# ishine/TTS-3

Measured on AMD Instinct MI355X. Metric: audio samples/sec + RTF, HiFiGAN-v1 22.05kHz 80-mel, batch 32 @ 1/2/4/8 GPU, higher is better.
Workload: dtype fp32 (power-of-2 scaled fp16 hi/lo split on fp16 MFMA, fp32 accumulate); 1 GPU; HiFiGAN-v1 22.05kHz inference, [32,80,1024] mel per GPU (replicate pad 5), fp32; model=HiFiGAN-v1 (hifigan_config.py generator_model_params), global_batch=32, seq_len=1024, parallelism=dp1 (utterance sharding; no collectives)

## Files before the change

tts-3_amd/csrc/kernels_resblock.hip:

```cpp
#include <algorithm>
#include <cstdlib>
#include <type_traits>

#include "resblock_block.hpp"
#include "split_device.hpp"

namespace tts {




constexpr int kPostK = 7;
constexpr int kPostHalo = 3;

template <class S, int K, int C, int PD, int GEO, bool ALLX = false, bool POST = false>
struct PairCfg {
  static constexpr int RP_W = (GEO == 0 || GEO == 4 || GEO == 5 || GEO == 7) ? 256 : (GEO == 1 ? 192 : 128);
  static constexpr int LEAD = (K - 1) / 2;
  static constexpr int RP_BN = RP_W - 2 * LEAD;
  static constexpr int NW = GEO >= 5 ? 8 : 4;
  static constexpr int NT = 64 * NW;
  static constexpr int WN = (GEO == 0 || GEO == 5) ? 4 : (GEO == 8 ? 1 : 2);
  static constexpr int WM = NW / WN;
  static constexpr int TM = C / 32 / WM;
// ... 186 lines not shown

  const int xrow0 = wn * TN * 32 + l32;
  auto read_x = [&](const unsigned char* xl, int k, f32x4 (*dst)[NP]) {
#pragma unroll
    for (int n = 0; n < TN; ++n) {
      const unsigned char* p = xl + (xrow0 + n * 32 + k * d) * S::ROWB + 16 * half;
#pragma unroll
      for (int q = 0; q < NP; ++q) dst[n][q] = *reinterpret_cast<const f32x4*>(p + 32 * q);
    }
  };

  if constexpr (ALLX) {
#pragma unroll
    for (int c = 0; c < NC; ++c) load_x(c);
#pragma unroll
    for (int c = 0; c < NC; ++c) store_x(c, c);
  } else {
    load_x(0);
    store_x(0, 0);
  }
  if (tid < C) {
    bsm[tid] = bias1;
    bsm[C + tid] = bias2;
  }
  if constexpr (POST)
    for (int e = tid; e < C * kPostK; e += NT) pws[e] = pa.post_w[e];
  __syncthreads();
#pragma unroll
  for (int c = 0; c < NC; ++c) {
    const unsigned char* xl = smem + (ALLX ? c : (c & 1)) * P::XSZB;
    if (!ALLX && c + 1 < NC) load_x(c + 1);
    read_x(xl, 0, bcur);
#pragma unroll
    for (int k = 0; k < K; ++k) {
      const int s = c * K + k;
#pragma unroll
      for (int m = 0; m < TM; ++m)
#pragma unroll
        for (int q = 0; q < NP; ++q) ar[PD][m][q] = bload4(ra[m], avoff, (unsigned)((s + PD) * NP + q) * 1024u);
      if (k + 1 < K) read_x(xl, k + 1, bnext);
      __builtin_amdgcn_sched_barrier(0);
      mfma_step();
      if (k + 1 < K) {
#pragma unroll
        for (int n = 0; n < TN; ++n)
#pragma unroll
          for (int q = 0; q < NP; ++q) bcur[n][q] = bnext[n][q];
      }
    }
    if (!ALLX && c + 1 < NC) store_x((c + 1) & 1, c + 1);
    if (!ALLX || c + 1 == NC) __syncthreads();
  }

  {
    const float sc1 = H3 ? ldexpf(1.f, ex + a1.w_exp) : 1.f;
    float tmax = 0.f;
#pragma unroll
    for (int m = 0; m < TM; ++m) {
      float bv[16];
#pragma unroll
      for (int r = 0; r < 16; ++r) bv[r] = bsm[mrow0 + m * 32 + (r & 3) + 8 * (r >> 2) + 4 * half];
#pragma unroll
      for (int n = 0; n < TN; ++n) {
        const int t = tx0 + xrow0 + n * 32;
        const bool inside = t >= 0 && t < T;
#pragma unroll
        for (int r = 0; r < 16; ++r) {
          float v = lrelu2(acc[m][n][r] * sc1 + bv[r], a1.out_slope);
          v = inside ? v : 0.f;
          acc[m][n][r] = v;
          tmax = fmaxf(tmax, fabsf(v));
        }
      }
    }
    float tscale = 1.f;
    int et = 0;
    if (H3) {
      tmax = wave_max(tmax);
      if (lane == 0) red[wave] = tmax;
      __syncthreads();
      float mx = red[0];
#pragma unroll
      for (int w = 1; w < P::NW; ++w) mx = fmaxf(mx, red[w]);
      if (mx > 0.f && mx < INFINITY) {
        int E;
        (void)frexpf(mx, &E);
        et = E - 14;
      }
      tscale = ldexpf(1.f, -et);
    }
#pragma unroll
    for (int m = 0; m < TM; ++m)
#pragma unroll
      for (int n = 0; n < TN; ++n)
#pragma unroll
        for (int gl = 0; gl < 2; ++gl)
          store_xt8<S>(smem + (((mrow0 + m * 32) / 16 + gl) * P::TROWS + xrow0 + n * 32) * S::ROWB + 16 * half,
                       acc[m][n], 8 * gl, tscale);
    constexpr int ZB = (P::TROWS - RP_W) * S::ROWB;
    for (int e = tid * 16; e < NC * ZB; e += NT * 16) {
      const int g = e / ZB;
      *reinterpret_cast<f32x4*>(smem + (g * P::TROWS + RP_W) * S::ROWB + (e - g * ZB)) = f32x4{};
    }
    __syncthreads();
    const Conv1dArgs& a2 = pa.c2;
#pragma unroll
    for (int m = 0; m < TM; ++m) ra[m] = make_rsrc(a2.w + ((size_t)(wm * TM + m) * NC * K) * (NP * 256), 0xFFFFFFFFu);
#pragma unroll
    for (int m = 0; m < TM; ++m)
#pragma unroll
      for (int n = 0; n < TN; ++n) acc[m][n] = f32x16{};
#pragma unroll
    for (int p = 0; p < PD; ++p)
#pragma unroll
      for (int m = 0; m < TM; ++m)
#pragma unroll
        for (int q = 0; q < NP; ++q) ar[p][m][q] = bload4(ra[m], avoff, (unsigned)(p * NP + q) * 1024u);
    const int trow0 = xrow0;
    auto read_t = [&](int g, int k, f32x4 (*dst)[NP]) {
#pragma unroll
      for (int n = 0; n < TN; ++n) {
        const unsigned char* p = smem + (g * P::TROWS + trow0 + n * 32 + k) * S::ROWB + 16 * half;
#pragma unroll
        for (int q = 0; q < NP; ++q) dst[n][q] = *reinterpret_cast<const f32x4*>(p + 32 * q);
      }
    };
    read_t(0, 0, bcur);
#pragma unroll
    for (int g = 0; g < NC; ++g) {
#pragma unroll
      for (int k = 0; k < K; ++k) {
        const int s = g * K + k;
#pragma unroll
        for (int m = 0; m < TM; ++m)
#pragma unroll
          for (int q = 0; q < NP; ++q) ar[PD][m][q] = bload4(ra[m], avoff, (unsigned)((s + PD) * NP + q) * 1024u);
        const bool more = (k + 1 < K) || (g + 1 < NC);
        if (more) read_t((k + 1 < K) ? g : g + 1, (k + 1 < K) ? k + 1 : 0, bnext);
        __builtin_amdgcn_sched_barrier(0);
        mfma_step();
        if (more) {
#pragma unroll
          for (int n = 0; n < TN; ++n)
#pragma unroll
            for (int q = 0; q < NP; ++q) bcur[n][q] = bnext[n][q];
        }
      }
    }
    if (H3) {
      const float sc2 = ldexpf(1.f, et + a2.w_exp);
#pragma unroll
      for (int m = 0; m < TM; ++m)
#pragma unroll
        for (int n = 0; n < TN; ++n) acc[m][n] *= sc2;
    }
    if constexpr (POST) {
      post_epilogue(pa, acc, b, t0, mrow0, wn, lane);
    } else {
      conv_epilogue<TM, TN, H3, YB>(a2, acc, b, t0 + wn * TN * 32, mrow0, lane, t0 + RP_BN, bsm + C);
    }
  }
}

namespace {
template <class S, int K, int C, int GEO>
void launch_pair_t(const ResPairArgs& a, int B, hipStream_t s) {
  constexpr bool AX = C == 64 && GEO != 2;
  constexpr int PD = S::NP == 1 ? RES_PD_B1 : 2;
  auto go = [&](auto pl_tag) {
    constexpr int PL = decltype(pl_tag)::value;
    if (a.post_w) {
      using P = PairCfg<S, K, C, PD, GEO, AX, true>;
      static_assert(P::RP_BN - 2 * kPostHalo <= 256, "one conv_post column per thread");
      dim3 grid(ceil_div(a.c1.Tout, P::STRIDE), 1, B);
      hipLaunchKernelGGL((resblock_pair_kernel<S, K, C, PD, GEO, AX, true, PL>), grid, dim3(P::NT), 0, s, a);
      return;
    }
    using P = PairCfg<S, K, C, PD, GEO, AX>;
    dim3 grid(ceil_div(a.c1.Tout, P::RP_BN), 1, B);
    hipLaunchKernelGGL((resblock_pair_kernel<S, K, C, PD, GEO, AX, false, PL>), grid, dim3(P::NT), 0, s, a);
  };
  if (a.c1.planes != 0) {
    constexpr bool OK = std::is_same<S, SchemeB1>::value;
    TTS_REQUIRE(OK && a.c1.planes == (kPlaneXB16 | kPlaneYB16) && a.c2.planes == a.c1.planes, 3,
                "resblock pair: bf16 planes need the bf16 scheme");
    if constexpr (OK) go(std::integral_constant<int, kPlaneXB16 | kPlaneYB16>{});
    return;
  }
  go(std::integral_constant<int, 0>{});
}

int pair_geo64() {
  static const int g = [] {
    const char* e = std::getenv("TTS_MI355X_PAIR_GEO64");
    return e && std::atoi(e) == 2 ? 2 : (e && std::atoi(e) == 4 ? 4 : 1);
  }();
  return g;
}

template <class S, int K>
void launch_pair_k(const ResPairArgs& a, int B, int C, hipStream_t s) {
  if constexpr (S::NP == 1) {
    if (C == 128) {
      static const int geo = [] {
        const char* e = std::getenv("TTS_MI355X_PAIR128_GEO");
        return e && e[0] == '2' ? 2 : (e && e[0] == '0' ? 0 : (e && e[0] == '4' ? 4 : (e && e[0] == '5' ? 5 : 7)));
      }();
      if (geo == 2) launch_pair_t<S, K, 128, 2>(a, B, s);
      else if (geo == 7) launch_pair_t<S, K, 128, 7>(a, B, s);
      else if (geo == 5) launch_pair_t<S, K, 128, 5>(a, B, s);
      else if (geo == 4) launch_pair_t<S, K, 128, 4>(a, B, s);
      else launch_pair_t<S, K, 128, 0>(a, B, s);
      return;
    }
    if (C == 256) {
      static const int geo = [] {
        const char* e = std::getenv("TTS_MI355X_PAIR256_GEO");
        return e && e[0] == '2' ? 2 : (e && e[0] == '6' ? 6 : 8);
      }();
      if (geo == 6) launch_pair_t<S, K, 256, 6>(a, B, s);
      else if (geo == 8) launch_pair_t<S, K, 256, 8>(a, B, s);
      else launch_pair_t<S, K, 256, 2>(a, B, s);
      return;
    }
  }
  if (C == 32) launch_pair_t<S, K, 32, 0>(a, B, s);
  else if (C == 64 && pair_geo64() == 2 && S::ROWB <= 80) launch_pair_t<S, K, 64, 2>(a, B, s);
  else if (C == 64 && pair_geo64() == 4 && S::NP == 1) launch_pair_t<S, K, 64, 4>(a, B, s);
  else if (C == 64) launch_pair_t<S, K, 64, 1>(a, B, s);
  else throw Error(3, "resblock pair: channels must be 32 or 64");
}

template <class S>
void launch_pair_s(const ResPairArgs& a, int B, int K, int C, hipStream_t s) {
  switch (K) {
    case 3: launch_pair_k<S, 3>(a, B, C, s); break;
    case 7: launch_pair_k<S, 7>(a, B, C, s); break;
    case 11: launch_pair_k<S, 11>(a, B, C, s); break;
    default: throw Error(3, "resblock pair: kernel size must be 3, 7 or 11");
  }
}
}

bool resblock_pair_supported(int mode, int C, int K, int dil) {
  return is_split_mode(mode) && (C == 32 || C == 64 || ((C == 128 || C == 256) && mode == MATH_BF16)) &&
         (K == 3 || K == 7 || K == 11) && dil >= 1 && dil <= 5;
}

bool resblock_pair128(int mode, int C, int K) {
  if (mode != MATH_BF16) return false;
  const char* e128 = std::getenv("TTS_MI355X_PAIR128");
  const char* e256 = std::getenv("TTS_MI355X_PAIR256");
  if (C == 128) return (K == 7 || K == 11) && !(e128 && e128[0] == '0');
  if (C == 256) {
    const char* e11 = std::getenv("TTS_MI355X_PAIR256_K11");
    return (K == 3 || K == 7 || (K == 11 && e11 && e11[0] == '1')) && !(e256 && e256[0] == '0');
  }
  return false;
}

bool resblock_pair_preferred(int mode, int C, int K, int dil) {
  return resblock_pair_supported(mode, C, K, dil);
}

void launch_resblock_pair(int mode, const ResPairArgs& a, int B, int K, int C, hipStream_t s) {
  TTS_REQUIRE(resblock_pair_supported(mode, C, K, a.c1.dil), 3, "resblock pair: unsupported configuration");
  TTS_REQUIRE(a.c1.Cin == C && a.c1.Cout == C && a.c2.Cin == C && a.c2.Cout == C && a.c1.Tin == a.c1.Tout &&
                  a.c2.Tout == a.c1.Tout && a.c1.rep_pad == 0 && a.c2.dil == 1,
              1, "resblock pair: bad arguments");
  TTS_REQUIRE(a.c2.res != a.c2.y || a.c2.zmode != 0, 1, "resblock pair: x and x' must not alias");
  TTS_REQUIRE(a.c1.cvec == nullptr && a.c2.cvec == nullptr && a.c1.bias && a.c2.bias, 1,
              "resblock pair: biases required, no cond vector (both are staged in LDS)");
  TTS_REQUIRE((int64_t)C * a.c1.Tout * 4 < (int64_t(1) << 31), 3, "resblock pair: plane exceeds 2 GiB");
  TTS_REQUIRE(!a.post_w || (a.c2.zmode == 3 && a.c2.res && a.c2.z && a.wav && !a.c2.mask), 1,
              "resblock pair: the fused conv_post needs the final MRF sum (zmode 3) with a residual");
  if (mode == MATH_FP32_F16X3) launch_pair_s<SchemeH3>(a, B, K, C, s);
  else if (mode == MATH_BF16) launch_pair_s<SchemeB1>(a, B, K, C, s);
  else launch_pair_s<SchemeX6>(a, B, K, C, s);
  TTS_HIP_CHECK(hipGetLastError());
}


namespace {
template <class S, int C, int GEO, int K>
void launch_res3_t(const ResBlock3Args& a, int B, hipStream_t s) {
  using P = Res3Cfg<S, C, GEO, K, 6, r3_xoff(K), r3_lead(K)>;
  dim3 grid(ceil_div(a.T, P::RP_BN), 1, B);
  launch_block_pl<S, C, GEO, K, 6, r3_xoff(K), r3_lead(K)>(a, grid, P::NT, s);
}
template <class S>
void launch_res3_s(const ResBlock3Args& a, int B, int C, int K, hipStream_t s) {
  if (K == 7) {
    if (C == 32) launch_res3_t<S, 32, 0, 7>(a, B, s);
    else launch_res3_t<S, 64, 0, 7>(a, B, s);
    return;
  }
  if (K == 11) {
    if (C == 32) launch_res3_t<S, 32, 0, 11>(a, B, s);
    else launch_res3_t<S, 64, 0, 11>(a, B, s);
    return;
  }
  if (C == 32) launch_res3_t<S, 32, 0, 3>(a, B, s);
  else if (C == 128) {
    if constexpr (S::ROWB <= 80) launch_res3_t<S, 128, 3, 3>(a, B, s);
    else throw Error(3, "resblock3: 128 channels need a split scheme of at most 80-byte rows");
  } else launch_res3_t<S, 64, 2, 3>(a, B, s);
}
}

bool resblock3_supported(int mode, int C, int K, const int* dil) {
  if (!is_split_mode(mode)) return false;
  if (K == 3) {
    if (!(C == 32 || C == 64 || (C == 128 && mode != MATH_FP32_X6))) return false;
  } else if (K == 7 || K == 11) {
    if (!(C == 32 || C == 64)) return false;
  } else {
    return false;
  }
  const int hk = (K - 1) / 2;
  int lo = -r3_xoff(K);
  for (int m = 0; m < 3; ++m) {
    if (dil[m] < 1 || hk * dil[m] > r3_xoff(K)) return false;
    lo = std::max(lo + hk * dil[m], 0) + hk;
  }
  return lo <= r3_lead(K);
}

void launch_resblock3(int mode, const ResBlock3Args& a, int B, int C, int K, hipStream_t s) {
  TTS_REQUIRE(resblock3_supported(mode, C, K, a.dil), 3, "resblock3: unsupported configuration");
  TTS_REQUIRE(a.zmode >= 1 && a.zmode <= 3 && a.z && a.x && a.x != a.z, 1, "resblock3: bad arguments");
  TTS_REQUIRE((int64_t)C * a.T * 4 < (int64_t(1) << 31), 3, "resblock3: plane exceeds 2 GiB");
  if (mode == MATH_FP32_F16X3) launch_res3_s<SchemeH3>(a, B, C, K, s);
  else if (mode == MATH_BF16) launch_res3_s<SchemeB1>(a, B, C, K, s);
  else launch_res3_s<SchemeX6>(a, B, C, K, s);
  TTS_HIP_CHECK(hipGetLastError());
}

bool resblock2_supported(int mode, int C, int K, const int* dil) {
  if (!is_split_mode(mode) || !(K == 3 || K == 5 || K == 7 || K == 11)) return false;
  if (!(C == 32 || C == 64 || (C == 128 && mode != MATH_FP32_X6 && (K == 3 || K == 5)))) return false;
  const int H = rb2_halo(K), hk = (K - 1) / 2;
  int lo = -H;
  for (int m = 0; m < 2; ++m) {
    if (dil[m] < 1 || hk * dil[m] > H) return false;
    lo = std::max(lo + hk * dil[m], 0);
  }
  return lo <= H;
}

bool resblock2_preferred(int mode, int C, int K, const int* dil) {
  if (!resblock2_supported(mode, C, K, dil)) return false;
  const char* e = std::getenv("TTS_MI355X_RB2_ALL");
  if (e && e[0] == '1') return true;
  return mode == MATH_BF16 || !(C == 64 && K == 11);
}

int resblock2_geo64(int mode) {
  const char* e = std::getenv("TTS_MI355X_RB2_GEO64");
  if (e && (e[0] == '0' || e[0] == '1')) return e[0] - '0';
  return mode == MATH_BF16 ? 1 : 0;
}

void launch_resblock2(int mode, const ResBlock3Args& a, int B, int C, int K, int geo64, hipStream_t s) {
  TTS_REQUIRE(resblock2_supported(mode, C, K, a.dil), 3, "resblock2: unsupported configuration");
  TTS_REQUIRE(a.zmode >= 1 && a.zmode <= 3 && a.z && a.x && a.x != a.z, 1, "resblock2: bad arguments");
  TTS_REQUIRE((int64_t)C * a.T * 4 < (int64_t(1) << 31), 3, "resblock2: plane exceeds 2 GiB");
  if (mode == MATH_FP32_F16X3) launch_resblock2_h3(a, B, C, K, geo64, s);
  else if (mode == MATH_BF16) launch_resblock2_b1(a, B, C, K, geo64, s);
  else launch_resblock2_x6(a, B, C, K, geo64, s);
  TTS_HIP_CHECK(hipGetLastError());
}

}
```

tts-3_amd/csrc/resblock_block.hpp:

```cpp
#pragma once
#include <type_traits>

#include "split_device.hpp"

#ifndef RES_PD_B1
#define RES_PD_B1 2
#endif
#ifndef RES_STAGE_8R
#define RES_STAGE_8R 1
#endif

namespace tts {

#ifndef R3_XR_POL
#define R3_XR_POL 0
#endif
constexpr int R3_XOFF = 5;
constexpr int R3_LEAD = 12;
constexpr int r3_xoff(int K) { return R3_XOFF * ((K - 1) / 2); }
constexpr int r3_lead(int K) { return R3_LEAD * ((K - 1) / 2); }
constexpr int rb2_halo(int K) { return K == 3 ? 4 : (K == 5 ? 12 : (K == 7 ? 9 : 15)); }

template <class S, int C, int GEO, int K = 3, int NCV = 6, int XO = R3_XOFF, int LEAD = R3_LEAD>
struct Res3Cfg {
  static constexpr int RP_W = GEO == 0 ? 256 : (GEO == 1 ? 192 : 128);
  static constexpr int RP_BN = RP_W - 2 * LEAD;
  static constexpr int NW = GEO == 3 ? 8 : 4;
  static constexpr int NT = 64 * NW;
  static constexpr int WN = GEO == 0 ? 4 : 2;
  static constexpr int WM = NW / WN;
  static constexpr int TM = C / 32 / WM;
  static constexpr int TN = RP_W / 32 / WN;
  static constexpr int NC = C / 16;
  static constexpr int PR = RP_W + 2 * XO;
  static constexpr int LDSB = NC * PR * S::ROWB;
  static_assert(TM >= 1 && TM * WM * 32 == C && TN * WN * 32 == RP_W, "geometry");
};

#ifndef RB3_W_B1
#define RB3_W_B1 0
#endif
#ifndef RB3_W64
#define RB3_W64 2
#endif
template <class S, int C, int GEO, int K, int NCV, int XO, int LEAD, int PL = 0>
__global__ __launch_bounds__((Res3Cfg<S, C, GEO, K, NCV, XO, LEAD>::NT))
__attribute__((amdgpu_waves_per_eu(S::NP == 1 && RB3_W_B1 > 0 ? RB3_W_B1
                                                                : (C == 64 && GEO == 2 ? RB3_W64 : (C == 32 || GEO == 3 ? 2 : 1)))))
void resblock3_kernel(ResBlock3Args a) {
  constexpr bool XB = (PL & kPlaneXB16) != 0, YB = (PL & kPlaneYB16) != 0;
  using PX = PlaneT<XB>;
  using PY = PlaneT<YB>;
  using P = Res3Cfg<S, C, GEO, K, NCV, XO, LEAD>;
  static_assert(NCV == 6 || NCV == 2, "ResBlock1 (6 convs) or ResBlock2 (2 convs)");
  constexpr int NP = S::NP;
  constexpr bool H3 = S::SCALED;
  constexpr int TM = P::TM, TN = P::TN, NC = P::NC, PR = P::PR, RP_W = P::RP_W;
  constexpr int PD = S::NP == 1 ? RES_PD_B1 : 2;
  __shared__ __attribute__((aligned(16))) unsigned char smem[P::LDSB];
  constexpr int NT = P::NT;
  __shared__ float red[2][P::NW];
  __shared__ float bsm[NCV * C];

  const int tid = threadIdx.x;
  const int lane = tid & 63;
  const int wave = tid >> 6;
  const int half = lane >> 5;
  const int l32 = lane & 31;
  const int wm = __builtin_amdgcn_readfirstlane(wave / P::WN);
  const int wn = wave % P::WN;
  const int mrow0 = wm * TM * 32;
  const int t0 = blockIdx.x * P::RP_BN;
  const int b = blockIdx.z;
  const int T = a.T;
  const int tx0 = t0 - LEAD;
  const int xcol0 = wn * TN * 32 + l32;
  const unsigned avoff = (unsigned)lane * 16u;
  const unsigned chb = (unsigned)T * PX::ES;
  const rsrc_t rx = make_rsrc(plane_at<XB>(a.x, (size_t)b * C * T), (unsigned)C * chb);
  auto ldx = [&](unsigned off, auto pol_tag) -> float {
    if constexpr (XB) return PX::ld(rx, off, 0u);
    else return bload_x<decltype(pol_tag)::value>(rx, off, 0u);
  };

  int ex = H3 ? amax_exp(a.amax_in, b) : 0;
  f32x16 xr[TM][TN];
  {
    const float xs = H3 ? ldexpf(1.f, -ex) : 1.f;
    constexpr int UG = (PR * 4 + NT - 1) / NT;
    constexpr int BPT = (C + NT - 1) / NT;
    float bl[NCV][BPT];
#pragma unroll
    for (int i = 0; i < NCV; ++i)
#pragma unroll
      for (int j = 0; j < BPT; ++j) {
        const int e = tid + j * NT;
        bl[i][j] = e < C ? a.bias[i][e] : 0.f;
      }
    f32x4 xv[NC][UG];
#pragma unroll
    for (int g = 0; g < NC; ++g)
#pragma unroll
      for (int i = 0; i < UG; ++i) {
        const int u = tid + i * NT;
        const int q = RES_STAGE_8R ? quad_pos((u >> 3) & 3) : (u & 3);
        const int r = RES_STAGE_8R ? (u >> 5) * 8 + (u & 7) : (u >> 2);
        const int ts = tx0 - XO + r;
        const bool ok = r < PR && ts >= 0 && ts < T;
        const unsigned vo = (unsigned)(16 * g + 4 * q) * chb + (unsigned)ts * PX::ES;
#pragma unroll
        for (int j = 0; j < 4; ++j)
          xv[g][i][j] = ldx(ok ? vo + (unsigned)j * chb : OOB_OFF, std::integral_constant<int, TTS_LDX_POL>{});
      }
    auto load_xr = [&] {
#pragma unroll
      for (int m = 0; m < TM; ++m)
#pragma unroll
        for (int n = 0; n < TN; ++n) {
          const int t = tx0 + xcol0 + n * 32;
          const bool tok = t >= 0 && t < T;
#pragma unroll
          for (int r = 0; r < 16; ++r) {
            const int co = mrow0 + m * 32 + (r & 3) + 8 * (r >> 2) + 4 * half;
            xr[m][n][r] = ldx(tok ? (unsigned)co * chb + (unsigned)t * PX::ES : OOB_OFF,
                              std::integral_constant<int, R3_XR_POL>{});
          }
        }
    };
#pragma unroll
    for (int g = 0; g < NC; ++g)
#pragma unroll
      for (int i = 0; i < UG; ++i) {
        const int u = tid + i * NT;
        const int q = RES_STAGE_8R ? quad_pos((u >> 3) & 3) : (u & 3);
        const int r = RES_STAGE_8R ? (u >> 5) * 8 + (u & 7) : (u >> 2);
        if (r < PR) {
          float v[4];
#pragma unroll
          for (int j = 0; j < 4; ++j) {
            v[j] = lrelu2(xv[g][i][j], 0.1f);
            if (H3) v[j] *= xs;
          }
          split_store4<S>(smem + (g * PR + r) * S::ROWB + 8 * quad_pos(q), v[0], v[1], v[2], v[3]);
        }
      }
    __builtin_amdgcn_sched_barrier(0);
    load_xr();
#pragma unroll
    for (int i = 0; i < NCV; ++i)
#pragma unroll
      for (int j = 0; j < BPT; ++j) {
        const int e = tid + j * NT;
        if (e < C) bsm[i * C + e] = bl[i][j];
      }
  }
  __syncthreads();

  f32x16 acc[TM][TN];
  f32x4 ar[PD + 1][TM][NP], bcur[TN][NP], bnext[TN][NP];
  rsrc_t ra[TM];
  auto conv = [&](int wi, int roff, int kstep) {
#pragma unroll
    for (int m = 0; m < TM; ++m) ra[m] = make_rsrc(a.w[wi] + ((size_t)(wm * TM + m) * NC * K) * (NP * 256), 0xFFFFFFFFu);
#pragma unroll
    for (int m = 0; m < TM; ++m)
#pragma unroll
      for (int n = 0; n < TN; ++n) acc[m][n] = f32x16{};
#pragma unroll
    for (int p = 0; p < PD; ++p)
#pragma unroll
      for (int m = 0; m < TM; ++m)
#pragma unroll
        for (int q = 0; q < NP; ++q) ar[p][m][q] = bload4(ra[m], avoff, (unsigned)(p * NP + q) * 1024u);
    auto read_b = [&](int g, int k, f32x4 (*dst)[NP]) {
#pragma unroll
      for (int n = 0; n < TN; ++n) {
        const unsigned char* pp = smem + (g * PR + xcol0 + n * 32 + roff + k * kstep) * S::ROWB + 16 * half;
#pragma unroll
        for (int q = 0; q < NP; ++q) dst[n][q] = *reinterpret_cast<const f32x4*>(pp + 32 * q);
      }
    };
    read_b(0, 0, bcur);
#pragma unroll
    for (int g = 0; g < NC; ++g) {
#pragma unroll
      for (int k = 0; k < K; ++k) {
        const int st = g * K + k;
#pragma unroll
        for (int m = 0; m < TM; ++m)
#pragma unroll
          for (int q = 0; q < NP; ++q)
            ar[PD][m][q] = bload4(ra[m], avoff, (unsigned)((st + PD) * NP + q) * 1024u);
        const bool more = (k + 1 < K) || (g + 1 < NC);
        if (more) read_b((k + 1 < K) ? g : g + 1, (k + 1 < K) ? k + 1 : 0, bnext);
        __builtin_amdgcn_sched_barrier(0);
#pragma unroll
        for (int e = 0; e < S::NPROD; ++e)
#pragma unroll
          for (int m = 0; m < TM; ++m)
#pragma unroll
            for (int n = 0; n < TN; ++n)
              acc[m][n] = S::mfma(ar[0][m][S::PA[e]], bcur[n][S::PB[e]], acc[m][n]);
#pragma unroll
        for (int p = 0; p < PD; ++p)
#pragma unroll
          for (int m = 0; m < TM; ++m)
#pragma unroll
            for (int q = 0; q < NP; ++q) ar[p][m][q] = ar[p + 1][m][q];
        if (more) {
#pragma unroll
          for (int n = 0; n < TN; ++n)
#pragma unroll
            for (int q = 0; q < NP; ++q) bcur[n][q] = bnext[n][q];
        }
      }
    }
  };
  int red_half = 0;
  auto tile_exp = [&](float vmax) -> int {
    if (!H3) return 0;
    vmax = wave_max(vmax);
    if (lane == 0) red[red_half][wave] = vmax;
    __syncthreads();
    float mx = red[red_half][0];
#pragma unroll
    for (int w = 1; w < P::NW; ++w) mx = fmaxf(mx, red[red_half][w]);
    red_half ^= 1;
    int e = 0;
    if (mx > 0.f && mx < INFINITY) {
      int E;
      (void)frexpf(mx, &E);
      e = E - 14;
    }
    return e;
  };

  auto store_pieces = [&](int roff, float scale) {
#pragma unroll
    for (int m = 0; m < TM; ++m)
#pragma unroll
      for (int n = 0; n < TN; ++n)
#pragma unroll
        for (int gl = 0; gl < 2; ++gl)
          store_xt8<S>(smem + (((mrow0 + m * 32) / 16 + gl) * PR + xcol0 + n * 32 + roff) * S::ROWB + 16 * half,
                       acc[m][n], 8 * gl, scale);
    constexpr int EB = 2 * XO * S::ROWB;
    for (int e = tid * 16; e < NC * EB; e += NT * 16) {
      const int g = e / EB;
      const int o = e - g * EB;
      const int lead_b = roff * S::ROWB;
      const int tail_b = (PR - roff - RP_W) * S::ROWB;
      if (o < lead_b) *reinterpret_cast<f32x4*>(smem + g * PR * S::ROWB + o) = f32x4{};
      else if (o - lead_b < tail_b)
        *reinterpret_cast<f32x4*>(smem + (g * PR + roff + RP_W) * S::ROWB + (o - lead_b)) = f32x4{};
    }
  };

  constexpr int HK = (K - 1) / 2;
  int lo = -XO, hi = RP_W + XO;
  auto residual_to_lds = [&](int ci) {
    const float sc = H3 ? ldexpf(1.f, ex + a.w_exp[ci]) : 1.f;
    const float* bs = bsm + ci * C;
    float vmax = 0.f;
#pragma unroll
    for (int m = 0; m < TM; ++m) {
      float bv[16];
#pragma unroll
      for (int r = 0; r < 16; ++r) bv[r] = bs[mrow0 + m * 32 + (r & 3) + 8 * (r >> 2) + 4 * half];
#pragma unroll
      for (int n = 0; n < TN; ++n) {
        const int col = xcol0 + n * 32;
        const int t = tx0 + col;
        const bool ok = col >= lo && col < hi && t >= 0 && t < T;
#pragma unroll
        for (int r = 0; r < 16; ++r) {
          const float x1 = (acc[m][n][r] * sc + bv[r]) + xr[m][n][r];
          xr[m][n][r] = x1;
          const float v = ok ? lrelu2(x1, 0.1f) : 0.f;
          acc[m][n][r] = v;
          vmax = fmaxf(vmax, fabsf(v));
        }
      }
    }
    const int e2 = tile_exp(vmax);
    if (!H3) __syncthreads();
    store_pieces(XO, H3 ? ldexpf(1.f, -e2) : 1.f);
    __syncthreads();
    ex = e2;
  };
  auto final_to_z = [&](int ci) {
    const float sc = H3 ? ldexpf(1.f, ex + a.w_exp[ci]) : 1.f;
    const float* bs = bsm + ci * C;
    const unsigned chbz = (unsigned)T * PY::ES;
    const rsrc_t rz = make_rsrc(plane_at<YB>(a.z, (size_t)b * C * T), (unsigned)C * chbz);
    float vmax = 0.f;
#pragma unroll
    for (int m = 0; m < TM; ++m) {
      float bv[16];
#pragma unroll
      for (int r = 0; r < 16; ++r) bv[r] = bs[mrow0 + m * 32 + (r & 3) + 8 * (r >> 2) + 4 * half];
#pragma unroll
      for (int n = 0; n < TN; ++n) {
        const int col = xcol0 + n * 32;
        const int t = tx0 + col;
        const bool keep = col >= LEAD && col < LEAD + P::RP_BN && t >= 0 && t < T;
        unsigned vo[16];
        float zv[16];
#pragma unroll
        for (int r = 0; r < 16; ++r) {
          const int co = mrow0 + m * 32 + (r & 3) + 8 * (r >> 2) + 4 * half;
          vo[r] = keep ? (unsigned)co * chbz + (unsigned)t * PY::ES : OOB_OFF;
          zv[r] = a.zmode >= 2 ? PY::ld(rz, vo[r], 0u) : 0.f;
        }
#pragma unroll
        for (int r = 0; r < 16; ++r) {
          float v = (acc[m][n][r] * sc + bv[r]) + xr[m][n][r];
          if (a.zmode == 2) v = zv[r] + v;
          else if (a.zmode == 3) v = (zv[r] + v) / a.zdiv;
          if (keep) vmax = fmaxf(vmax, fabsf(v));
          PY::st(rz, v, vo[r], 0u);
        }
      }
    }
    if (H3 && a.amax_out) publish_amax(a.amax_out, b, vmax);
  };

  if constexpr (NCV == 6) {
#pragma unroll 1
    for (int it = 0; it < 3; ++it) {
      const int d = a.dil[it];
      conv(2 * it, XO - HK * d, d);
      lo = max(lo + HK * d, 0);
      hi = min(hi - HK * d, RP_W);
      {
        const float sc = H3 ? ldexpf(1.f, ex + a.w_exp[2 * it]) : 1.f;
        const float* bs = bsm + (2 * it) * C;
        float vmax = 0.f;
#pragma unroll
        for (int m = 0; m < TM; ++m) {
          float bv[16];
#pragma unroll
          for (int r = 0; r < 16; ++r) bv[r] = bs[mrow0 + m * 32 + (r & 3) + 8 * (r >> 2) + 4 * half];
#pragma unroll
          for (int n = 0; n < TN; ++n) {
            const int col = xcol0 + n * 32;
            const int t = tx0 + col;
            const bool ok = col >= lo && col < hi && t >= 0 && t < T;
#pragma unroll
            for (int r = 0; r < 16; ++r) {
              float v = lrelu2(acc[m][n][r] * sc + bv[r], 0.1f);
              v = ok ? v : 0.f;
              acc[m][n][r] = v;
              vmax = fmaxf(vmax, fabsf(v));
            }
          }
        }
        const int et = tile_exp(vmax);
        if (!H3) __syncthreads();
        store_pieces(HK, H3 ? ldexpf(1.f, -et) : 1.f);
        __syncthreads();
        ex = et;
      }
      conv(2 * it + 1, 0, 1);
      lo += HK;
      hi -= HK;
      if (it < 2) residual_to_lds(2 * it + 1);
      else final_to_z(2 * it + 1);
    }
  } else {
#pragma unroll 1
    for (int it = 0; it < 2; ++it) {
      const int d = a.dil[it];
      conv(it, XO - HK * d, d);
      lo = max(lo + HK * d, 0);
      hi = min(hi - HK * d, RP_W);
      if (it == 0) residual_to_lds(0);
      else final_to_z(1);
    }
  }
}

}

namespace tts {
template <class S, int C, int GEO, int K, int NCV, int XO, int LEAD>
void launch_block_pl(const ResBlock3Args& a, dim3 grid, int nt, hipStream_t s) {
  if (a.planes != 0) {
    constexpr bool OK = std::is_same<S, SchemeB1>::value;
    TTS_REQUIRE(OK && a.planes == (kPlaneXB16 | kPlaneYB16), 3, "resblock block: bf16 planes need the bf16 scheme");
    if constexpr (OK)
      hipLaunchKernelGGL((resblock3_kernel<S, C, GEO, K, NCV, XO, LEAD, kPlaneXB16 | kPlaneYB16>), grid, dim3(nt), 0, s, a);
    return;
  }
  hipLaunchKernelGGL((resblock3_kernel<S, C, GEO, K, NCV, XO, LEAD>), grid, dim3(nt), 0, s, a);
}
template <class S, int C, int GEO, int K>
void launch_rb2_t(const ResBlock3Args& a, int B, hipStream_t s) {
  constexpr int H = rb2_halo(K);
  using P = Res3Cfg<S, C, GEO, K, 2, H, H>;
  dim3 grid(ceil_div(a.T, P::RP_BN), 1, B);
  launch_block_pl<S, C, GEO, K, 2, H, H>(a, grid, P::NT, s);
}
template <class S, int C, int GEO>
void launch_rb2_k(const ResBlock3Args& a, int B, int K, hipStream_t s) {
  if (K == 3) launch_rb2_t<S, C, GEO, 3>(a, B, s);
  else if (K == 5) launch_rb2_t<S, C, GEO, 5>(a, B, s);
  else if (K == 7) launch_rb2_t<S, C, GEO, 7>(a, B, s);
  else launch_rb2_t<S, C, GEO, 11>(a, B, s);
}
template <class S>
void launch_rb2_s(const ResBlock3Args& a, int B, int C, int K, int geo64, hipStream_t s) {
  if (C == 32) launch_rb2_k<S, 32, 0>(a, B, K, s);
  else if (C == 64) {
    if (geo64 == 1) launch_rb2_k<S, 64, 1>(a, B, K, s);
    else launch_rb2_k<S, 64, 2>(a, B, K, s);
  } else {
    if constexpr (S::ROWB <= 80) {
      if (K == 3) launch_rb2_t<S, 128, 3, 3>(a, B, s);
      else launch_rb2_t<S, 128, 3, 5>(a, B, s);
    } else {
      throw Error(3, "resblock2: 128 channels need a split scheme of at most 80-byte rows");
    }
  }
}
void launch_resblock2_h3(const ResBlock3Args& a, int B, int C, int K, int geo64, hipStream_t s);
void launch_resblock2_b1(const ResBlock3Args& a, int B, int C, int K, int geo64, hipStream_t s);
void launch_resblock2_x6(const ResBlock3Args& a, int B, int C, int K, int geo64, hipStream_t s);
}
```

tts-3_amd/csrc/split_device.hpp:

```cpp
#pragma once

#include "conv_device.hpp"

namespace tts {

typedef __bf16 bf16x8 __attribute__((ext_vector_type(8)));
typedef _Float16 f16x8 __attribute__((ext_vector_type(8)));
typedef unsigned short u16x4 __attribute__((ext_vector_type(4)));
typedef unsigned u32x2 __attribute__((ext_vector_type(2)));

__device__ __forceinline__ unsigned short bf16_bits(__bf16 h) { return __builtin_bit_cast(unsigned short, h); }
__device__ __forceinline__ unsigned short f16_bits(_Float16 h) { return __builtin_bit_cast(unsigned short, h); }

struct SchemeX6 {
  static constexpr int NP = 3;
  static constexpr int ROWB = 112;
  static constexpr int NACC = 1;
  static constexpr int NPROD = 6;
  static constexpr int PA[6] = {2, 1, 0, 1, 0, 0};
  static constexpr int PB[6] = {0, 1, 2, 0, 1, 0};
  static constexpr int PACC[6] = {0, 0, 0, 0, 0, 0};
  static constexpr bool SCALED = false;
  __device__ static __forceinline__ void split(float x, unsigned short (&p)[3]) {
    const __bf16 a0 = (__bf16)x;
    const float r1 = x - (float)a0;
    const __bf16 a1 = (__bf16)r1;
    const float r2 = r1 - (float)a1;
    p[0] = bf16_bits(a0);
    p[1] = bf16_bits(a1);
    p[2] = bf16_bits((__bf16)r2);
  }
  __device__ static __forceinline__ void split2(float x0, float x1, unsigned (&w)[3]) {
    unsigned short a[3], b[3];
    split(x0, a);
    split(x1, b);
#pragma unroll
    for (int p = 0; p < 3; ++p) w[p] = (unsigned)a[p] | ((unsigned)b[p] << 16);
  }
  __device__ static __forceinline__ f32x16 mfma(f32x4 a, f32x4 b, f32x16 c) {
    return __builtin_amdgcn_mfma_f32_32x32x16_bf16(__builtin_bit_cast(bf16x8, a), __builtin_bit_cast(bf16x8, b), c, 0, 0, 0);
  }
};

struct SchemeH3 {
  static constexpr int NP = 2;
  static constexpr int ROWB = 80;
  static constexpr int NACC = 1;
  static constexpr int NPROD = 3;
  static constexpr int PA[3] = {1, 0, 0};
  static constexpr int PB[3] = {0, 1, 0};
  static constexpr int PACC[3] = {0, 0, 0};
  static constexpr bool SCALED = true;
  __device__ static __forceinline__ void split(float x, unsigned short (&p)[2]) {
    const _Float16 h = (_Float16)x;
    p[0] = f16_bits(h);
    p[1] = f16_bits((_Float16)(x - (float)h));
  }
  __device__ static __forceinline__ void split2(float x0, float x1, unsigned (&w)[2]) {
    typedef float f2 __attribute__((ext_vector_type(2)));
    typedef _Float16 h2 __attribute__((ext_vector_type(2)));
    const h2 h = __builtin_convertvector((f2){x0, x1}, h2);
    const unsigned hb = __builtin_bit_cast(unsigned, h);
    float r0, r1;
    asm("v_fma_mix_f32 %0, -%1, 1.0, %2 op_sel_hi:[1,0,0]" : "=v"(r0) : "v"(hb), "v"(x0));
    asm("v_fma_mix_f32 %0, -%1, 1.0, %2 op_sel:[1,0,0] op_sel_hi:[1,0,0]" : "=v"(r1) : "v"(hb), "v"(x1));
    w[0] = hb;
    w[1] = __builtin_bit_cast(unsigned, __builtin_convertvector((f2){r0, r1}, h2));
  }
  __device__ static __forceinline__ f32x16 mfma(f32x4 a, f32x4 b, f32x16 c) {
    return __builtin_amdgcn_mfma_f32_32x32x16_f16(__builtin_bit_cast(f16x8, a), __builtin_bit_cast(f16x8, b), c, 0, 0, 0);
  }
};

struct SchemeB1 {
  static constexpr int NP = 1;
  static constexpr int ROWB = 48;
  static constexpr int NACC = 1;
  static constexpr int NPROD = 1;
  static constexpr int PA[1] = {0};
  static constexpr int PB[1] = {0};
  static constexpr int PACC[1] = {0};
  static constexpr bool SCALED = false;
  __device__ static __forceinline__ void split(float x, unsigned short (&p)[1]) { p[0] = bf16_bits((__bf16)x); }
  __device__ static __forceinline__ void split2(float x0, float x1, unsigned (&w)[1]) {
    w[0] = (unsigned)bf16_bits((__bf16)x0) | ((unsigned)bf16_bits((__bf16)x1) << 16);
  }
  __device__ static __forceinline__ f32x16 mfma(f32x4 a, f32x4 b, f32x16 c) {
    return __builtin_amdgcn_mfma_f32_32x32x16_bf16(__builtin_bit_cast(bf16x8, a), __builtin_bit_cast(bf16x8, b), c, 0, 0, 0);
  }
};

template <class S>
__device__ __forceinline__ void split_store4(unsigned char* dst, float v0, float v1, float v2, float v3) {
  unsigned w0[S::NP], w1[S::NP];
  S::split2(v0, v1, w0);
  S::split2(v2, v3, w1);
#pragma unroll
  for (int p = 0; p < S::NP; ++p) *reinterpret_cast<u32x2*>(dst + 32 * p) = u32x2{w0[p], w1[p]};
}

template <class S, class V>
__device__ __forceinline__ void store_xt8(unsigned char* dst, const V& acc, int r0, float scale) {
  unsigned w[4][S::NP];
#pragma unroll
  for (int k = 0; k < 4; ++k) S::split2(acc[r0 + 2 * k] * scale, acc[r0 + 2 * k + 1] * scale, w[k]);
#pragma unroll
  for (int p = 0; p < S::NP; ++p)
    *reinterpret_cast<u32x4_t*>(dst + 32 * p) = u32x4_t{w[0][p], w[1][p], w[2][p], w[3][p]};
}

__device__ __forceinline__ int amax_exp(const unsigned* slots, int b) {
  if (!slots) return 0;
  float m = __uint_as_float(slots[(size_t)b * 64 + (threadIdx.x & 63)]);
  m = wave_max(m);
  int e = 0;
  if (m > 0.f && m < INFINITY) {
    int E;
    (void)frexpf(m, &E);
    e = E - 14;
  }
  return __builtin_amdgcn_readfirstlane(e);
}

}
```

Measured before the change: 164.0 million samples/s.

## Add swizzled 64-byte LDS rows and 2-WG/CU geometry for 128-channel ResBlock1

```diff
diff --git a/tts-3_amd/csrc/kernels_resblock.hip b/tts-3_amd/csrc/kernels_resblock.hip
--- a/tts-3_amd/csrc/kernels_resblock.hip
+++ b/tts-3_amd/csrc/kernels_resblock.hip
@@ -512,7 +512,8 @@
   }
   if (C == 32) launch_res3_t<S, 32, 0, 3>(a, B, s);
   else if (C == 128) {
-    if constexpr (S::ROWB <= 80) launch_res3_t<S, 128, 3, 3>(a, B, s);
+    if constexpr (S::NP == 2) launch_res3_t<S, 128, 4, 3>(a, B, s);
+    else if constexpr (S::ROWB <= 80) launch_res3_t<S, 128, 3, 3>(a, B, s);
     else throw Error(3, "resblock3: 128 channels need a split scheme of at most 80-byte rows");
   } else launch_res3_t<S, 64, 2, 3>(a, B, s);
 }
diff --git a/tts-3_amd/csrc/res3_layout.hpp b/tts-3_amd/csrc/res3_layout.hpp
--- /dev/null
+++ b/tts-3_amd/csrc/res3_layout.hpp
@@ -0,0 +1,16 @@
+#pragma once
+
+namespace tts {
+
+template <int NP, bool SWZ>
+struct Res3Rows {
+  static_assert(!SWZ || NP == 2, "the swizzle permutes the 4 units of a two-piece row");
+  static constexpr int UNITS = 2 * NP;
+  static constexpr int PITCH = SWZ ? 32 * NP : 32 * NP + 16;
+  static constexpr int unit(int row, int lu) { return SWZ ? (lu ^ ((row >> 2) & 3)) : lu; }
+  static constexpr int off(int row, int lu) { return row * PITCH + 16 * unit(row, lu); }
+  static constexpr int piece(int off0, int q) { return SWZ ? (off0 ^ (32 * q)) : off0 + 32 * q; }
+  static constexpr bool SWIZZLED = SWZ;
+};
+
+}
diff --git a/tts-3_amd/csrc/resblock_block.hpp b/tts-3_amd/csrc/resblock_block.hpp
--- a/tts-3_amd/csrc/resblock_block.hpp
+++ b/tts-3_amd/csrc/resblock_block.hpp
@@ -1,6 +1,7 @@
 #pragma once
 #include <type_traits>
 
+#include "res3_layout.hpp"
 #include "split_device.hpp"
 
 #ifndef RES_PD_B1
@@ -33,7 +34,11 @@
   static constexpr int TN = RP_W / 32 / WN;
   static constexpr int NC = C / 16;
   static constexpr int PR = RP_W + 2 * XO;
-  static constexpr int LDSB = NC * PR * S::ROWB;
+  using ROWS = Res3Rows<S::NP, GEO == 4 && S::NP == 2>;
+  static_assert(GEO == 4 || ROWS::PITCH == S::ROWB, "the padded layout is the scheme's own row");
+  static constexpr int LDSB = NC * PR * ROWS::PITCH;
+  static constexpr int LDS_TOTAL = LDSB + 2 * NW * 4 + NCV * C * 4;
+  static_assert(GEO != 4 || LDS_TOTAL <= 80 * 1024, "GEO 4: two workgroups per CU");
   static_assert(TM >= 1 && TM * WM * 32 == C && TN * WN * 32 == RP_W, "geometry");
 };
 
@@ -46,12 +51,13 @@
 template <class S, int C, int GEO, int K, int NCV, int XO, int LEAD, int PL = 0>
 __global__ __launch_bounds__((Res3Cfg<S, C, GEO, K, NCV, XO, LEAD>::NT))
 __attribute__((amdgpu_waves_per_eu(S::NP == 1 && RB3_W_B1 > 0 ? RB3_W_B1
-                                                                : (C == 64 && GEO == 2 ? RB3_W64 : (C == 32 || GEO == 3 ? 2 : 1)))))
+                                                                : (C == 64 && GEO == 2 ? RB3_W64 : (C == 32 || GEO >= 3 ? 2 : 1)))))
 void resblock3_kernel(ResBlock3Args a) {
   constexpr bool XB = (PL & kPlaneXB16) != 0, YB = (PL & kPlaneYB16) != 0;
   using PX = PlaneT<XB>;
   using PY = PlaneT<YB>;
   using P = Res3Cfg<S, C, GEO, K, NCV, XO, LEAD>;
+  using ROWS = typename P::ROWS;
   static_assert(NCV == 6 || NCV == 2, "ResBlock1 (6 convs) or ResBlock2 (2 convs)");
   constexpr int NP = S::NP;
   constexpr bool H3 = S::SCALED;
@@ -78,10 +84,11 @@
   const unsigned avoff = (unsigned)lane * 16u;
   const unsigned chb = (unsigned)T * PX::ES;
   const rsrc_t rx = make_rsrc(plane_at<XB>(a.x, (size_t)b * C * T), (unsigned)C * chb);
-  auto ldx = [&](unsigned off, auto pol_tag) -> float {
-    if constexpr (XB) return PX::ld(rx, off, 0u);
-    else return bload_x<decltype(pol_tag)::value>(rx, off, 0u);
-  };
+  auto ldx = [&](unsigned off, auto pol_tag, unsigned soff = 0u) -> float {
+    if constexpr (XB) return PX::ld(rx, off, soff);
+    else return bload_x<decltype(pol_tag)::value>(rx, off, soff);
+  };
+  constexpr bool SOFF = GEO == 4;
 
   int ex = H3 ? amax_exp(a.amax_in, b) : 0;
   f32x16 xr[TM][TN];
@@ -119,11 +126,15 @@
         for (int n = 0; n < TN; ++n) {
           const int t = tx0 + xcol0 + n * 32;
           const bool tok = t >= 0 && t < T;
+          const unsigned vlane = tok ? (unsigned)(4 * half) * chb + (unsigned)t * PX::ES : OOB_OFF;
 #pragma unroll
           for (int r = 0; r < 16; ++r) {
             const int co = mrow0 + m * 32 + (r & 3) + 8 * (r >> 2) + 4 * half;
-            xr[m][n][r] = ldx(tok ? (unsigned)co * chb + (unsigned)t * PX::ES : OOB_OFF,
-                              std::integral_constant<int, R3_XR_POL>{});
+            if constexpr (SOFF)
+              xr[m][n][r] = ldx(vlane, std::integral_constant<int, R3_XR_POL>{}, (unsigned)(co - 4 * half) * chb);
+            else
+              xr[m][n][r] = ldx(tok ? (unsigned)co * chb + (unsigned)t * PX::ES : OOB_OFF,
+                                std::integral_constant<int, R3_XR_POL>{});
           }
         }
     };
@@ -141,7 +152,11 @@
             v[j] = lrelu2(xv[g][i][j], 0.1f);
             if (H3) v[j] *= xs;
           }
-          split_store4<S>(smem + (g * PR + r) * S::ROWB + 8 * quad_pos(q), v[0], v[1], v[2], v[3]);
+          const int qp = quad_pos(q);
+          unsigned char* dst[NP];
+#pragma unroll
+          for (int p = 0; p < NP; ++p) dst[p] = smem + ROWS::off(g * PR + r, (qp >> 1) + 2 * p) + 8 * (qp & 1);
+          split_store4<S>(dst, v[0], v[1], v[2], v[3]);
         }
       }
     __builtin_amdgcn_sched_barrier(0);
@@ -159,7 +174,8 @@
   f32x16 acc[TM][TN];
   f32x4 ar[PD + 1][TM][NP], bcur[TN][NP], bnext[TN][NP];
   rsrc_t ra[TM];
-  auto conv = [&](int wi, int roff, int kstep) {
+  auto conv = [&](int wi, int roff, int kstep) __attribute__((always_inline)) {
+    if constexpr (ROWS::SWIZZLED) asm volatile("" : "+s"(roff), "+s"(kstep));
 #pragma unroll
     for (int m = 0; m < TM; ++m) ra[m] = make_rsrc(a.w[wi] + ((size_t)(wm * TM + m) * NC * K) * (NP * 256), 0xFFFFFFFFu);
 #pragma unroll
@@ -172,12 +188,13 @@
       for (int m = 0; m < TM; ++m)
 #pragma unroll
         for (int q = 0; q < NP; ++q) ar[p][m][q] = bload4(ra[m], avoff, (unsigned)(p * NP + q) * 1024u);
-    auto read_b = [&](int g, int k, f32x4 (*dst)[NP]) {
+    auto read_b = [&](int g, int k, f32x4 (*dst)[NP]) __attribute__((always_inline)) {
 #pragma unroll
       for (int n = 0; n < TN; ++n) {
-        const unsigned char* pp = smem + (g * PR + xcol0 + n * 32 + roff + k * kstep) * S::ROWB + 16 * half;
-#pragma unroll
-        for (int q = 0; q < NP; ++q) dst[n][q] = *reinterpret_cast<const f32x4*>(pp + 32 * q);
+        const int o = ROWS::off(g * PR + xcol0 + roff + k * kstep, half);
+#pragma unroll
+        for (int q = 0; q < NP; ++q)
+          dst[n][q] = *reinterpret_cast<const f32x4*>(smem + ROWS::piece(o, q) + n * 32 * ROWS::PITCH);
       }
     };
     read_b(0, 0, bcur);
@@ -217,7 +234,7 @@
     }
   };
   int red_half = 0;
-  auto tile_exp = [&](float vmax) -> int {
+  auto tile_exp = [&](float vmax) __attribute__((always_inline)) -> int {
     if (!H3) return 0;
     vmax = wave_max(vmax);
     if (lane == 0) red[red_half][wave] = vmax;
@@ -235,30 +252,36 @@
     return e;
   };
 
-  auto store_pieces = [&](int roff, float scale) {
+  auto store_pieces = [&](int roff, float scale) __attribute__((always_inline)) {
+    if constexpr (ROWS::SWIZZLED) asm volatile("" : "+s"(roff));
 #pragma unroll
     for (int m = 0; m < TM; ++m)
 #pragma unroll
       for (int n = 0; n < TN; ++n)
 #pragma unroll
-        for (int gl = 0; gl < 2; ++gl)
-          store_xt8<S>(smem + (((mrow0 + m * 32) / 16 + gl) * PR + xcol0 + n * 32 + roff) * S::ROWB + 16 * half,
-                       acc[m][n], 8 * gl, scale);
-    constexpr int EB = 2 * XO * S::ROWB;
+        for (int gl = 0; gl < 2; ++gl) {
+          const int o = ROWS::off(((mrow0 + m * 32) / 16 + gl) * PR + xcol0 + roff, half);
+          unsigned char* dst[NP];
+#pragma unroll
+          for (int p = 0; p < NP; ++p) dst[p] = smem + ROWS::piece(o, p) + n * 32 * ROWS::PITCH;
+          store_xt8<S>(dst, acc[m][n], 8 * gl, scale);
+        }
+    constexpr int ROWB = ROWS::PITCH;
+    constexpr int EB = 2 * XO * ROWB;
     for (int e = tid * 16; e < NC * EB; e += NT * 16) {
       const int g = e / EB;
       const int o = e - g * EB;
-      const int lead_b = roff * S::ROWB;
-      const int tail_b = (PR - roff - RP_W) * S::ROWB;
-      if (o < lead_b) *reinterpret_cast<f32x4*>(smem + g * PR * S::ROWB + o) = f32x4{};
+      const int lead_b = roff * ROWB;
+      const int tail_b = (PR - roff - RP_W) * ROWB;
+      if (o < lead_b) *reinterpret_cast<f32x4*>(smem + g * PR * ROWB + o) = f32x4{};
       else if (o - lead_b < tail_b)
-        *reinterpret_cast<f32x4*>(smem + (g * PR + roff + RP_W) * S::ROWB + (o - lead_b)) = f32x4{};
+        *reinterpret_cast<f32x4*>(smem + (g * PR + roff + RP_W) * ROWB + (o - lead_b)) = f32x4{};
     }
   };
 
   constexpr int HK = (K - 1) / 2;
   int lo = -XO, hi = RP_W + XO;
-  auto residual_to_lds = [&](int ci) {
+  auto residual_to_lds = [&](int ci) __attribute__((always_inline)) {
     const float sc = H3 ? ldexpf(1.f, ex + a.w_exp[ci]) : 1.f;
     const float* bs = bsm + ci * C;
     float vmax = 0.f;
@@ -288,7 +311,7 @@
     __syncthreads();
     ex = e2;
   };
-  auto final_to_z = [&](int ci) {
+  auto final_to_z = [&](int ci) __attribute__((always_inline)) {
     const float sc = H3 ? ldexpf(1.f, ex + a.w_exp[ci]) : 1.f;
     const float* bs = bsm + ci * C;
     const unsigned chbz = (unsigned)T * PY::ES;
@@ -304,13 +327,19 @@
         const int col = xcol0 + n * 32;
         const int t = tx0 + col;
         const bool keep = col >= LEAD && col < LEAD + P::RP_BN && t >= 0 && t < T;
-        unsigned vo[16];
+        unsigned vo[16], so[16];
         float zv[16];
 #pragma unroll
         for (int r = 0; r < 16; ++r) {
           const int co = mrow0 + m * 32 + (r & 3) + 8 * (r >> 2) + 4 * half;
-          vo[r] = keep ? (unsigned)co * chbz + (unsigned)t * PY::ES : OOB_OFF;
-          zv[r] = a.zmode >= 2 ? PY::ld(rz, vo[r], 0u) : 0.f;
+          if constexpr (SOFF) {
+            vo[r] = keep ? (unsigned)(4 * half) * chbz + (unsigned)t * PY::ES : OOB_OFF;
+            so[r] = (unsigned)(co - 4 * half) * chbz;
+          } else {
+            vo[r] = keep ? (unsigned)co * chbz + (unsigned)t * PY::ES : OOB_OFF;
+            so[r] = 0u;
+          }
+          zv[r] = a.zmode >= 2 ? PY::ld(rz, vo[r], so[r]) : 0.f;
         }
 #pragma unroll
         for (int r = 0; r < 16; ++r) {
@@ -318,7 +347,7 @@
           if (a.zmode == 2) v = zv[r] + v;
           else if (a.zmode == 3) v = (zv[r] + v) / a.zdiv;
           if (keep) vmax = fmaxf(vmax, fabsf(v));
-          PY::st(rz, v, vo[r], 0u);
+          PY::st(rz, v, vo[r], so[r]);
         }
       }
     }
@@ -326,8 +355,8 @@
   };
 
   if constexpr (NCV == 6) {
-#pragma unroll 1
-    for (int it = 0; it < 3; ++it) {
+    auto iteration = [&](int it, auto last_tag) __attribute__((always_inline)) {
+      constexpr int LAST = decltype(last_tag)::value;
       const int d = a.dil[it];
       conv(2 * it, XO - HK * d, d);
       lo = max(lo + HK * d, 0);
@@ -364,8 +393,16 @@
       conv(2 * it + 1, 0, 1);
       lo += HK;
       hi -= HK;
-      if (it < 2) residual_to_lds(2 * it + 1);
+      if (LAST == 1 || (LAST == 0 && it < 2)) residual_to_lds(2 * it + 1);
       else final_to_z(2 * it + 1);
+    };
+    if constexpr (GEO == 4) {
+#pragma unroll 1
+      for (int it = 0; it < 2; ++it) iteration(it, std::integral_constant<int, 1>{});
+      iteration(2, std::integral_constant<int, 2>{});
+    } else {
+#pragma unroll 1
+      for (int it = 0; it < 3; ++it) iteration(it, std::integral_constant<int, 0>{});
     }
   } else {
 #pragma unroll 1
diff --git a/tts-3_amd/csrc/split_device.hpp b/tts-3_amd/csrc/split_device.hpp
--- a/tts-3_amd/csrc/split_device.hpp
+++ b/tts-3_amd/csrc/split_device.hpp
@@ -98,6 +98,14 @@
 #pragma unroll
   for (int p = 0; p < S::NP; ++p) *reinterpret_cast<u32x2*>(dst + 32 * p) = u32x2{w0[p], w1[p]};
 }
+template <class S>
+__device__ __forceinline__ void split_store4(unsigned char* const (&dst)[S::NP], float v0, float v1, float v2, float v3) {
+  unsigned w0[S::NP], w1[S::NP];
+  S::split2(v0, v1, w0);
+  S::split2(v2, v3, w1);
+#pragma unroll
+  for (int p = 0; p < S::NP; ++p) *reinterpret_cast<u32x2*>(dst[p]) = u32x2{w0[p], w1[p]};
+}
 
 template <class S, class V>
 __device__ __forceinline__ void store_xt8(unsigned char* dst, const V& acc, int r0, float scale) {
@@ -107,6 +115,15 @@
 #pragma unroll
   for (int p = 0; p < S::NP; ++p)
     *reinterpret_cast<u32x4_t*>(dst + 32 * p) = u32x4_t{w[0][p], w[1][p], w[2][p], w[3][p]};
+}
+template <class S, class V>
+__device__ __forceinline__ void store_xt8(unsigned char* const (&dst)[S::NP], const V& acc, int r0, float scale) {
+  unsigned w[4][S::NP];
+#pragma unroll
+  for (int k = 0; k < 4; ++k) S::split2(acc[r0 + 2 * k] * scale, acc[r0 + 2 * k + 1] * scale, w[k]);
+#pragma unroll
+  for (int p = 0; p < S::NP; ++p)
+    *reinterpret_cast<u32x4_t*>(dst[p]) = u32x4_t{w[0][p], w[1][p], w[2][p], w[3][p]};
 }
 
 __device__ __forceinline__ int amax_exp(const unsigned* slots, int b) {
diff --git a/tts-3_amd/tests_native/res3_layout_check.cpp b/tts-3_amd/tests_native/res3_layout_check.cpp
--- /dev/null
+++ b/tts-3_amd/tests_native/res3_layout_check.cpp
@@ -0,0 +1,155 @@
+#include <algorithm>
+#include <cstdio>
+#include <vector>
+
+#include "common.hpp"
+#include "res3_layout.hpp"
+
+using namespace tts;
+
+static int failures = 0;
+#define CHECK(cond, ...)                          \
+  do {                                            \
+    if (!(cond)) {                                \
+      if (failures < 20) {                        \
+        std::fprintf(stderr, "FAIL: " __VA_ARGS__); \
+        std::fprintf(stderr, "\n");               \
+      }                                           \
+      ++failures;                                 \
+    }                                             \
+  } while (0)
+
+constexpr int NC = 8, RP_W = 128, XO = 5, HK = 1, PR = RP_W + 2 * XO, ROWS_ALL = NC * PR;
+
+static int worst(const std::vector<int>& addr, const std::vector<int>& lanes, int dw, int banks) {
+  std::vector<std::vector<int>> on(banks);
+  for (int l : lanes) {
+    if (addr[l] < 0) continue;
+    for (int j = 0; j < dw; ++j) {
+      const int d = addr[l] / 4 + j;
+      auto& v = on[d % banks];
+      if (std::find(v.begin(), v.end(), d) == v.end()) v.push_back(d);
+    }
+  }
+  size_t w = 0;
+  for (const auto& v : on) w = std::max(w, v.size());
+  return (int)w;
+}
+
+static std::vector<std::vector<int>> read128_groups() {
+  const int a[2][16] = {{0, 1, 2, 3, 12, 13, 14, 15, 20, 21, 22, 23, 24, 25, 26, 27},
+                        {4, 5, 6, 7, 8, 9, 10, 11, 16, 17, 18, 19, 28, 29, 30, 31}};
+  std::vector<std::vector<int>> g;
+  for (int h = 0; h < 2; ++h)
+    for (int s = 0; s < 2; ++s) {
+      std::vector<int> v;
+      for (int i = 0; i < 16; ++i) v.push_back(a[s][i] + 32 * h);
+      g.push_back(v);
+    }
+  return g;
+}
+static std::vector<std::vector<int>> contiguous_groups(int n) {
+  std::vector<std::vector<int>> g;
+  for (int l0 = 0; l0 < 64; l0 += n) {
+    std::vector<int> v;
+    for (int i = 0; i < n; ++i) v.push_back(l0 + i);
+    g.push_back(v);
+  }
+  return g;
+}
+
+template <class R>
+static void check_map(const char* name) {
+  for (int row = 0; row < ROWS_ALL; ++row) {
+    bool seen[R::UNITS] = {};
+    for (int lu = 0; lu < R::UNITS; ++lu) {
+      const int pu = R::unit(row, lu);
+      CHECK(pu >= 0 && pu < R::UNITS && !seen[pu], "%s: row %d unit %d -> %d is no bijection", name, row, lu, pu);
+      if (pu >= 0 && pu < R::UNITS) seen[pu] = true;
+      CHECK(R::off(row, lu) >= row * R::PITCH && R::off(row, lu) + 16 <= (row + 1) * R::PITCH,
+            "%s: row %d unit %d leaves its row", name, row, lu);
+    }
+    for (int half = 0; half < 2; ++half)
+      for (int q = 0; q < R::UNITS / 2; ++q)
+        CHECK(R::piece(R::off(row, half), q) == R::off(row, half + 2 * q), "%s: piece() row %d", name, row);
+    for (int j = 1; row + 16 * j < ROWS_ALL && j <= 4; ++j)
+      for (int lu = 0; lu < R::UNITS; ++lu)
+        CHECK(R::off(row + 16 * j, lu) == R::off(row, lu) + 16 * j * R::PITCH, "%s: + 16 j rows, row %d", name, row);
+  }
+}
+
+template <class R>
+static void check_accesses(const char* name, int max_store) {
+  constexpr int NP = R::UNITS / 2;
+  const auto rg = read128_groups();
+  const auto w8 = contiguous_groups(8), w16 = contiguous_groups(16);
+  std::vector<int> addr(64);
+  struct Tap { int roff, kstep; };
+  std::vector<Tap> taps;
+  for (int d : {1, 3, 5}) taps.push_back({XO - HK * d, d});
+  taps.push_back({0, 1});
+  for (const Tap& t : taps)
+    for (int g = 0; g < NC; ++g)
+      for (int wn = 0; wn < 2; ++wn)
+        for (int n = 0; n < 2; ++n)
+          for (int k = 0; k < 3; ++k)
+            for (int q = 0; q < NP; ++q) {
+              for (int lane = 0; lane < 64; ++lane) {
+                const int row = g * PR + wn * 64 + (lane & 31) + n * 32 + t.roff + k * t.kstep;
+                CHECK(row >= g * PR && row < (g + 1) * PR, "%s: read row %d outside group %d", name, row, g);
+                addr[lane] = R::off(row, (lane >> 5) + 2 * q);
+              }
+              for (const auto& grp : rg)
+                CHECK(worst(addr, grp, 4, 64) == 1, "%s: ds_read_b128 conflict (roff %d kstep %d g %d wn %d n %d k %d q %d)",
+                      name, t.roff, t.kstep, g, wn, n, k, q);
+            }
+  for (int roff : {XO, HK})
+    for (int g = 0; g < NC; ++g)
+      for (int wn = 0; wn < 2; ++wn)
+        for (int n = 0; n < 2; ++n)
+          for (int p = 0; p < NP; ++p) {
+            for (int lane = 0; lane < 64; ++lane)
+              addr[lane] = R::off(g * PR + wn * 64 + (lane & 31) + n * 32 + roff, (lane >> 5) + 2 * p);
+            for (const auto& grp : w8)
+              CHECK(worst(addr, grp, 4, 32) <= max_store, "%s: ds_write_b128 conflict (roff %d g %d wn %d n %d p %d)",
+                    name, roff, g, wn, n, p);
+          }
+  for (int NT : {256, 512})
+    for (int g = 0; g < NC; ++g)
+      for (int u0 = 0; u0 < ((PR * 4 + NT - 1) / NT) * NT; u0 += 64)
+        for (int p = 0; p < NP; ++p) {
+          for (int lane = 0; lane < 64; ++lane) {
+            const int u = u0 + lane;
+            const int q = quad_pos((u >> 3) & 3), r = (u >> 5) * 8 + (u & 7), qp = quad_pos(q);
+            addr[lane] = r < PR ? R::off(g * PR + r, (qp >> 1) + 2 * p) + 8 * (qp & 1) : -1;
+          }
+          for (const auto& grp : w16)
+            CHECK(worst(addr, grp, 2, 32) <= max_store, "%s: ds_write_b64 conflict (NT %d g %d u0 %d p %d)", name, NT, g, u0, p);
+        }
+}
+
+int main() {
+  using Swz = Res3Rows<2, true>;
+  using Pad2 = Res3Rows<2, false>;
+  using Pad1 = Res3Rows<1, false>;
+  using Pad3 = Res3Rows<3, false>;
+  static_assert(Swz::PITCH == 64 && Pad2::PITCH == 80 && Pad1::PITCH == 48 && Pad3::PITCH == 112, "row pitches");
+  check_map<Swz>("swizzled");
+  check_map<Pad2>("padded f16x3");
+  check_map<Pad1>("padded bf16");
+  check_map<Pad3>("padded x6");
+  check_accesses<Pad2>("padded f16x3", 1);
+  check_accesses<Pad1>("padded bf16", 1);
+  check_accesses<Swz>("swizzled", 2);
+  {
+    std::vector<int> addr(64);
+    for (int lane = 0; lane < 64; ++lane) addr[lane] = ((lane & 31) + XO) * 64 + 16 * (lane >> 5);
+    CHECK(worst(addr, read128_groups()[0], 4, 64) == 4, "the replay does not see the 4-way conflict of plain 64-byte rows");
+  }
+  if (failures) {
+    std::fprintf(stderr, "%d layout check(s) failed\n", failures);
+    return 1;
+  }
+  std::printf("res3_layout_check: maps are bijections, reads conflict-free, swizzled stores at most 2-way\n");
+  return 0;
+}
```

Result: faster. 165.9 million samples/s, median of 6 (+1.2%).
